# jydu/comap

Measured on AMD Instinct MI355X. Metric: site-pair coevolution statistics/s (incl. null sims), higher is better.
Workload: dtype f64; 1 GPU; target: north-star target: 10000x64 protein JTT92+G4(a=0.5), correlation, 1000 null replicates x 10000; observed_pairs=49995000, null_pairs_total=10000000, null_pairs_this_gpu=10000000, parallelism=single GPU, pair_output=compact, cu_count=256, mapping_waves=2048

## Files before the change

### comap_amd/csrc/cmx_api_ctx.cpp

```cpp
#include "cmx_ctx.h"

thread_local std::string g_create_error;

constexpr int kGuardByte = 0xC5;
std::atomic<int> g_guard{-1};
std::mutex g_guard_mu;
std::vector<std::string> g_guard_failures;
std::map<std::string, size_t> g_guard_shrink;

std::atomic<int> g_lds_slot{1};
std::atomic<int> g_pat_hash_bits{64};
std::atomic<int> g_map_queue{1};
std::atomic<int> g_map_small_blocks{1};
std::atomic<int> g_map_grid{0};

bool guard_on() {
  int g = g_guard.load();
  if (g < 0) {
    const char* e = getenv("CMX_SCRATCH_GUARD");
    g = (e && e[0] == '1') ? 1 : 0;
    g_guard.store(g);
  }
  return g == 1;
}

void guard_record(const std::string& what) {
  std::lock_guard<std::mutex> lk(g_guard_mu);
  g_guard_failures.push_back(what);
  std::fprintf(stderr, "CMX_SCRATCH_GUARD: %s\n", what.c_str());
}

hipError_t guard_arm(void* base, size_t logical) {
  return hipMemset(static_cast<char*>(base) + logical, kGuardByte, kGuardBytes);
}

bool guard_intact(const void* base, size_t logical, size_t* first_bad) {
// ... 173 lines not shown
      CMX_TRY(upload(ctx, h.MAT, &mat));
      d.MAT = const_cast<double*>(mat);
      d.MC = h.MC;
      auto up_stream = [&](const std::vector<int>& stream, const int** dev, int* nmv) -> cmx_status {
        std::vector<int> ms(stream);
        const int unit = mat_unit(h.dS);
        for (size_t i = 0; i < ms.size(); i += 2) ms[i] *= unit;
        const size_t n2 = ms.size();
        for (size_t i = 0; i < 4; ++i) ms.push_back(ms[i % n2]);
        *nmv = (int)(stream.size() / 2);
        return upload(ctx, ms, dev);
      };
      CMX_TRY(up_stream(h.msched, &d.msched, &d.nmv));
      d.msched_r = nullptr;
      d.nmv_r = 0;
      if (!h.msched_r.empty()) CMX_TRY(up_stream(h.msched_r, &d.msched_r, &d.nmv_r));
      d.plan = nullptr;
      if (!h.wait_imm.empty()) CMX_TRY(upload(ctx, planned_stream(h), &d.plan));
      UP(nrec);
    }
    UP(simg); UP(simord);
    d.nsimg = (int)(h.simg.size() / 16);
    UP(eigV); UP(eigVi); UP(eigLam); UP(model_of); UP(blen);
    UP(CP); UP(CPG); UP(pi); UP(rates); UP(probs); UP(cum_pi); UP(cum_probs);
#undef UP
    if (h.plain) return CMX_OK;
    HIP_TRY(ctx, launch_extend_leaf_rows(d, nullptr, nullptr));
    HIP_TRY(ctx, hipDeviceSynchronize());
    ctx->leaf_rows_custom = false;
    for (int i = 0; i < 256; ++i) dm[i] = i < h.S ? (1u << i) : ((h.S >= 32) ? 0xffffffffu : ((1u << h.S) - 1u));
    HIP_TRY(ctx, hipMemcpy(ctx->d_default_masks, dm.data(), sizeof(uint32_t) * 256, hipMemcpyHostToDevice));
    ctx->grid_blocks = ctx->cu_count * map_waves_per_simd(h.dS);
    ctx->waves = ctx->grid_blocks * kWavesPerBlock;
    ctx->obs_blocks = std::max(1, ctx->grid_blocks / 4);
    if (const int cap = g_map_grid.load()) {
      ctx->grid_blocks = std::min(ctx->grid_blocks, cap);
      ctx->waves = ctx->grid_blocks * kWavesPerBlock;
      ctx->obs_blocks = std::min(ctx->obs_blocks, cap);
    }
    auto alloc_ws = [&](Workspace* ws, size_t w, size_t* bytes) -> cmx_status {
      const size_t ks = (size_t)map_sites_per_wave(h.dS);
      const size_t bD = w * h.NIW * h.dS * ks * sizeof(double);
      const size_t bC = w * 2 * h.B * h.K * ks * sizeof(double);
      const size_t bP = w * h.dC * h.B * h.K * ks * sizeof(double);
      const bool g = guard_on();
      auto one = [&](const char* nm, void** p, size_t bytes) -> cmx_status {
// ... 101 lines not shown
}

cmx_status cmx_debug_wait_plan(const cmx_model* model, const cmx_tree* tree, int32_t* distance, int32_t* immediate, size_t cap, size_t* n) {
  HostModel hm;
  int code = CMX_OK;
  hm.lds_slot = g_lds_slot.load() != 0;
  const std::string msg = build_host_model(model, tree, &hm, &code);
  if (!msg.empty()) {
    g_create_error = msg;
    return (cmx_status)code;
  }
  if (hm.wait_imm.size() > cap) {
    g_create_error = "cmx_debug_wait_plan: buffers too small";
    return CMX_ERR_INVALID;
  }
  std::memcpy(distance, hm.wait_dist.data(), hm.wait_dist.size() * sizeof(int32_t));
  std::memcpy(immediate, hm.wait_imm.data(), hm.wait_imm.size() * sizeof(int32_t));
  *n = hm.wait_imm.size();
  return CMX_OK;
}

int cmx_debug_wait_skew(int entry) { return wait_plan_skew(entry); }

cmx_status cmx_synchronize(cmx_ctx* ctx) {
  if (!ctx) return CMX_ERR_INVALID;
  HIP_TRY(ctx, hipSetDevice(ctx->device));
  HIP_TRY(ctx, hipDeviceSynchronize());
  return guard_verify_all(ctx);
}

cmx_status cmx_scratch_check(cmx_ctx* ctx) {
  if (!ctx) return CMX_ERR_INVALID;
  if (!guard_on()) return fail(ctx, CMX_ERR_UNSUPPORTED, "the scratch guard is off (CMX_SCRATCH_GUARD=1 or cmx_debug_scratch_guard(1) before the context is created)");
  HIP_TRY(ctx, hipSetDevice(ctx->device));
  HIP_TRY(ctx, hipDeviceSynchronize());
  return guard_verify_all(ctx);
}

int cmx_debug_scratch_guard(int on) {
  const int was = guard_on() ? 1 : 0;
  if (on >= 0) g_guard.store(on ? 1 : 0);
  return was;
}

int cmx_debug_lds_slot(int on) {
  const int was = g_lds_slot.load();
  if (on >= 0) g_lds_slot.store(on ? 1 : 0);
  return was;
}

int cmx_debug_map_queue(int on) {
  const int was = g_map_queue.load();
  if (on >= 0) g_map_queue.store(on ? 1 : 0);
  return was;
}

int cmx_debug_map_small_blocks(int on) {
  const int was = g_map_small_blocks.load();
  if (on >= 0) g_map_small_blocks.store(on ? 1 : 0);
  return was;
}

int cmx_debug_map_grid(int workgroups) {
  const int was = g_map_grid.load();
  if (workgroups >= 0) g_map_grid.store(workgroups);
  return was;
}

size_t cmx_debug_scratch_guard_failures(char* buf, size_t cap, int clear) {
  std::lock_guard<std::mutex> lk(g_guard_mu);
  const size_t n = g_guard_failures.size();
  if (buf && cap) {
    std::string all;
    for (const std::string& f : g_guard_failures) { all += f; all += '\n'; }
    std::snprintf(buf, cap, "%s", all.c_str());
  }
// ... 78 lines not shown
```

### comap_amd/csrc/cmx_api_null.cpp

```cpp
#include "cmx_ctx.h"

constexpr size_t kNullAlnPassBytes = (size_t)4 << 30;
static size_t null_pass_bytes(size_t dflt) {
  static const size_t env = [] {
    const char* e = getenv("CMX_NULL_PASS_BYTES");
    return e ? (size_t)strtoull(e, nullptr, 10) : (size_t)0;
  }();
  return env ? env : dflt;
}

cmx_status cmx_null_simulate_dev(cmx_ctx* ctx, uint64_t seed, size_t rep_begin, size_t rep_end, size_t rep_ram, uint8_t* d_aln,
                                 void* stream) {
  CMX_TRY(need_model(ctx));
  if (rep_end <= rep_begin || rep_ram == 0 || !d_aln) return fail(ctx, CMX_ERR_INVALID, "cmx_null_simulate: bad arguments");
  CMX_TRY(rng_range(ctx, (uint64_t)rep_end * 2 * rep_ram, "cmx_null_simulate"));
  HIP_TRY(ctx, hipSetDevice(ctx->device));
  const size_t nsites = (rep_end - rep_begin) * 2 * rep_ram;
  const size_t chunk = std::min<size_t>(nsites, std::max<size_t>((size_t)1 << 21, (((size_t)4 << 30) / (size_t)ctx->hm.nn) & ~(size_t)1023));
  uint8_t* d_states;
  CMX_TRY(scratch(ctx, "null_states", (size_t)ctx->hm.nn * chunk, &d_states));
  HIP_TRY(ctx, launch_simulate_blocked(ctx->dm, seed, (uint64_t)rep_begin * 2 * rep_ram, nsites, rep_ram, d_aln, d_states, chunk,
                                       (hipStream_t)stream));
  return CMX_OK;
}

static cmx_status null_unfused_dev(cmx_ctx* ctx1, cmx_ctx* ctx2, int kind, const double* params, uint64_t seed,
                                   size_t rep_begin, size_t rep_end, size_t rep_ram, const uint8_t* d_supplied, double* d_stat,
                                   int32_t* d_rcmin, double* d_prmin, double* d_nmin, void* stream) {
  CMX_TRY(need_model(ctx1));
  if (!ctx2 || !ctx2->has_model) return fail(ctx1, CMX_ERR_INVALID, "cmx_null_inter: second context has no model");
  CMX_TRY(check_kind(ctx1, kind));
  if (rep_end <= rep_begin || rep_ram == 0 || !d_stat) return fail(ctx1, CMX_ERR_INVALID, "cmx_null_inter: bad arguments");
  CMX_TRY(rng_range(ctx1, (uint64_t)rep_end * 2 * rep_ram, "cmx_null_inter"));
  CMX_TRY(rng_range(ctx2, (uint64_t)rep_end * 2 * rep_ram, "cmx_null_inter"));
  if (ctx1->device != ctx2->device) return fail(ctx1, CMX_ERR_INVALID, "cmx_null_inter: contexts live on different devices");
  if (ctx1->hm.B != ctx2->hm.B || ctx1->hm.K != ctx2->hm.K)
    return fail(ctx1, CMX_ERR_INVALID, "cmx_null_inter: the two data sets must have the same branches and substitution types "
                                       "(Statistic::getValueForPair throws DimensionException otherwise)");
  HIP_TRY(ctx1, hipSetDevice(ctx1->device));
  hipStream_t st = (hipStream_t)stream;
  const size_t nrep = rep_end - rep_begin, n = nrep * rep_ram;
  const size_t BK = (size_t)ctx1->hm.B * ctx1->hm.K;
  double *cnt[2], *pr[2], *nm[2];
  int32_t* rc[2];
  cmx_ctx* cx[2] = {ctx1, ctx2};
// ... 261 lines not shown
```

### comap_amd/csrc/cmx_ctx.h

```cpp
#pragma once
#include <hip/hip_runtime.h>

#include <algorithm>
#include <atomic>
#include <cmath>
#include <cstdio>
#include <cstring>
#include <map>
#include <mutex>
#include <string>
#include <vector>

#include "../../include/comap_mi355x.h"
#include "cmx_device.h"
#include "cmx_host_model.h"

using namespace cmx;

#pragma GCC visibility push(hidden)

struct DevBuf {
  void* p = nullptr;
  size_t bytes = 0;
  size_t logical = 0;
// ... 5 lines not shown
  std::vector<long long> host;
  size_t M = 0;
  int sh = -1;
  size_t allocs = 0;
};

struct cmx_ctx {
  int device = 0;
  bool has_model = false;
  HostModel hm;
  DevModel dm{};
  Workspace ws{};
  Workspace ws_obs{};
  int obs_blocks = 0;
  int cu_count = 0, waves = 0, grid_blocks = 0;
  size_t ws_bytes = 0;
  unsigned long long* map_queue = nullptr;
  unsigned map_queue_turn = 0;
  std::vector<void*> model_allocs;
  std::map<std::string, DevBuf> scratch;
  struct GuardedFixed { std::string name; void* p; size_t bytes; };
  std::vector<GuardedFixed> guarded_fixed;
  uint32_t* d_default_masks = nullptr;
  unsigned stat_mean_turn = 0;
  std::vector<double> param_host[8];
  bool leaf_rows_custom = false;
  bool map_average = true;
  bool map_joint = true;
  bool scaling = false;
  std::vector<double> stat_w;
  double* d_stat_w = nullptr;
  std::vector<long long> perm_dF_host;
  std::vector<uint8_t> perm_tab_host;
  PermTable perm_F, permw_F;
  struct GramKept { bool valid = false; int kind = 0; const double* counts = nullptr; size_t n = 0, ldc = 0, row_begin = 0, row_end = 0; const double* stat = nullptr; } gram_kept;
  const double *va_P = nullptr, *va_N1 = nullptr, *va_NC = nullptr;
  const double *va_PN = nullptr, *va_pi = nullptr;
  const int *va_first = nullptr, *va_next = nullptr;
  WideOps va_wide{};
  const int* asr_inner = nullptr;
  int asr_n_inner = 0;
  int null_patterns = -1;
  int null_depth = 0;
  unsigned long long null_mapped_host = 0;
  bool null_mapped_dev = false;
  mutable std::string err;
// ... 2 lines not shown
#define CMX_TRY(expr)                                                                                        \
  do {                                                                                                       \
    cmx_status s_ = (expr);                                                                                  \
    if (s_ != CMX_OK) return s_;                                                                             \
  } while (0)

#define HIP_TRY(ctx, expr)                                                                                   \
  do {                                                                                                       \
    hipError_t e_ = (expr);                                                                                  \
    if (e_ != hipSuccess) {                                                                                  \
      (ctx)->err = std::string(#expr) + ": " + hipGetErrorString(e_);                                        \
      return CMX_ERR_DEVICE;                                                                                 \
    }                                                                                                        \
  } while (0)

extern thread_local std::string g_create_error;
extern std::atomic<int> g_guard;
extern std::mutex g_guard_mu;
extern std::vector<std::string> g_guard_failures;
extern std::map<std::string, size_t> g_guard_shrink;
extern std::atomic<int> g_pat_hash_bits;
extern std::atomic<int> g_map_queue;
extern std::atomic<int> g_map_small_blocks;
extern std::atomic<int> g_map_grid;

inline cmx_status fail(cmx_ctx* ctx, cmx_status s, const std::string& msg) {
  if (ctx) ctx->err = msg;
  return s;
}

inline cmx_status need_model(cmx_ctx* ctx) {
  if (!ctx) return CMX_ERR_INVALID;
  if (!ctx->has_model) return fail(ctx, CMX_ERR_INVALID, "this context was created without a model/tree");
  return CMX_OK;
}

template <class T>
cmx_status upload(cmx_ctx* ctx, const std::vector<T>& h, const T** d) {
  void* p = nullptr;
  const size_t bytes = sizeof(T) * (h.empty() ? 1 : h.size());
  HIP_TRY(ctx, hipMalloc(&p, bytes));
  ctx->model_allocs.push_back(p);
  if (!h.empty()) HIP_TRY(ctx, hipMemcpy(p, h.data(), sizeof(T) * h.size(), hipMemcpyHostToDevice));
  *d = static_cast<const T*>(p);
  return CMX_OK;
}
// ... 94 lines not shown
```

### comap_amd/csrc/cmx_device.h

```cpp
#pragma once
#include <hip/hip_runtime.h>

#include "../../include/comap_mi355x.h"
#include <stddef.h>
#include <stdint.h>

#include "cmx_layout.h"

namespace cmx {

constexpr int kWave = 64;
constexpr int kWavesPerBlock = 4;
constexpr int map_ng(int) { return 4; }
constexpr int map_sites_per_wave(int S) { return 16 * map_ng(S); }
constexpr int map_waves_per_simd(int S) { return S == 4 ? 3 : 2; }
constexpr bool map_lds_slot(int S, int fuse, int ng) { return S == 20 && fuse == 1 && ng == 4; }

struct DevModel {
  int S, C, K, nn, B, T, NI, NIW, NV, root;
  int S0, C0, fuse;
  const int* taxon_of;
  const int* parent;
  double* MAT;
  int MC;
// ... 92 lines not shown
inline int pair_Bp(int B) { return (B + 3) / 4 * 4; }
struct SiteCols { const int32_t* rc = nullptr; const double *pr = nullptr, *nm = nullptr; };
struct PairOut {
  double* stat = nullptr;
  int32_t* rcmin = nullptr;
  double *prmin = nullptr, *nmin = nullptr;
  PairOut at(size_t o) const { return {stat + o, rcmin ? rcmin + o : nullptr, prmin ? prmin + o : nullptr, nmin ? nmin + o : nullptr}; }
};
struct GramBatch { size_t nblk, zsite, zout, zx; };
struct RowScan { unsigned long long* rowcount = nullptr; void* tmp = nullptr; size_t tmp_bytes = 0; };

hipError_t launch_map(const MapArgs& a, int mode, int grid_blocks, hipStream_t stream);
hipError_t launch_map_queue_init(unsigned long long* queue, unsigned long long first, hipStream_t stream);
hipError_t launch_map_finalize(const MapArgs& a, hipStream_t stream);
hipError_t launch_extend_leaf_rows(const DevModel& m, const uint32_t* d_masks, hipStream_t stream);
hipError_t launch_pair_diag(const Stat& st, const double* c1, size_t ld1, const SiteCols& s1, const double* c2, size_t ld2,
                            const SiteCols& s2, size_t n, const PairOut& out, hipStream_t stream);
hipError_t launch_group_stats(const Stat& st, const double* d_counts, size_t ld, const int64_t* d_offsets, const int32_t* d_sites,
                              size_t ngroups, double* d_out, hipStream_t stream);
hipError_t launch_simulate(const DevModel& m, uint64_t seed, uint64_t g0, size_t n, uint8_t* d_aln, size_t ld,
                           int32_t* d_classes, uint8_t* d_states, hipStream_t stream, size_t rep_ram = 0, uint64_t gstep = 0);
hipError_t launch_simulate_continuous(const DevModel& m, uint64_t seed, uint64_t g0, size_t n, double alpha, double p_inv,
                                      uint8_t* d_aln, size_t ld, double* d_rates, uint8_t* d_states, hipStream_t stream);
hipError_t launch_simulate_blocked(const DevModel& m, uint64_t seed, uint64_t g0, size_t nsites, size_t blk, uint8_t* d_aln,
                                   uint8_t* d_states, size_t chunk, hipStream_t stream);
hipError_t launch_pair_prep(const Stat& st, const double* d_counts, size_t n, size_t ldc, const double* d_mvec, size_t blk,
                            const PairOperand& o, hipStream_t stream);
hipError_t launch_pair_gram(const Stat& st, const PairOperand& a, const PairOperand& b, PairMode mode, double* d_out, size_t ldo,
                            const GramBatch& z, size_t irow0, hipStream_t stream);
hipError_t launch_mi_classify(const Stat& st, const double* d_counts, size_t n, size_t ldc, const PairOperand& o, hipStream_t stream);
hipError_t launch_mi_pairs_block(int B, const PairOperand& a, const PairOperand& b, PairMode mode, double* d_out, size_t ldo,
                                 size_t irow0, hipStream_t stream);
hipError_t launch_mi_pairs_diag(int B, const PairOperand& a, const PairOperand& b, size_t n, double* d_out, hipStream_t stream);
hipError_t launch_mi_group(int B, const PairOperand& g, const int64_t* d_offsets, const int32_t* d_sites, size_t ngroups,
                           double* d_out, hipStream_t stream);
enum class PlainMode : int { NoAvg = 0 , Marginal = 1, NoAvgMarginal = 2 , Joint = 3 };
struct PlainArgs {
  int S, C, K, nn, B, root;
  PlainMode mode;
  int Sreal;
  const double* PN;
  const double* rates;
  double *logL, *post_rate;
  int32_t* rate_class;
  const int *first_child, *next_sib, *taxon_of, *parent;
  const double* P;
  const double* N1;
  const double* NC;
// ... 166 lines not shown
```

### comap_amd/csrc/cmx_host_model.cpp

```cpp
#include "cmx_host_parts.h"

#include <algorithm>
#include <cmath>
#include <cstring>

namespace cmx {
namespace {

using Mat = std::vector<double>;

Mat matmul(int n, const Mat& A, const Mat& B) {
  Mat C((size_t)n * n, 0.0);
  for (int i = 0; i < n; ++i)
    for (int k = 0; k < n; ++k) {
      const double a = A[(size_t)i * n + k];
      for (int j = 0; j < n; ++j) C[(size_t)i * n + j] += a * B[(size_t)k * n + j];
    }
  return C;
}

void jacobi(int n, Mat A, Mat* U, std::vector<double>* lam) {
  U->assign((size_t)n * n, 0.0);
  for (int i = 0; i < n; ++i) (*U)[(size_t)i * n + i] = 1.0;
  for (int sweep = 0; sweep < 200; ++sweep) {
// ... 308 lines not shown

void build_sim_tables(HostModel* hm) {
  const int S = hm->S, C = hm->C, B = hm->B, nn = hm->nn;
  const size_t S2 = (size_t)S * S;
  hm->CP.assign((size_t)C * nn * S2 + 4, 0.0);
  for (int c = 0; c < C; ++c)
    for (int b = 0; b < B; ++b) {
      const double* P = &hm->P[((size_t)c * B + b) * S2];
      double* cp = &hm->CP[((size_t)c * nn + b) * S2];
      for (int x = 0; x < S; ++x) {
        double cum = 0.0;
        for (int y = 0; y < S; ++y) { cum += P[(size_t)x * S + y]; cp[(size_t)x * S + y] = cum; }
      }
    }
  hm->CPG.assign((size_t)C * nn * S * 32, 0);
  for (size_t r = 0; r < (size_t)C * nn * S; ++r) {
    const double* cum = &hm->CP[r * S];
    for (int k = 0; k < 32; ++k) {
      int st = 0;
      while (st < S - 1 && cum[st] <= k / 32.0) ++st;
      hm->CPG[r * 32 + k] = (uint8_t)st;
    }
  }
  hm->cum_pi.resize(S);
  hm->cum_probs.resize(C);
  double cum = 0.0;
  for (int x = 0; x < S; ++x) { cum += hm->pi[x]; hm->cum_pi[x] = cum; }
  cum = 0.0;
  for (int c = 0; c < C; ++c) { cum += hm->probs[c]; hm->cum_probs[c] = cum; }
}

}

std::string build_host_model(const cmx_model* model, const cmx_tree* tree, HostModel* hm, int* code) {
  *code = CMX_ERR_INVALID;
  std::vector<Eig> eig;
  std::string bad = check_arguments(model, tree, hm, code);
  if (bad.empty()) bad = build_tree(tree, hm);
  if (!bad.empty()) return bad;
  build_walk_program(hm);
  build_sim_groups(hm);
  bad = check_model(model, hm);
  if (bad.empty()) bad = build_generators(model, hm, &eig);
  if (!bad.empty()) return bad;
  build_branch_matrices(model, eig, hm);
  build_device_matrices(hm);
// ... 10 lines not shown
```

### comap_amd/csrc/cmx_host_model.h

```cpp
#pragma once
#include <cstdint>
#include <string>
#include <vector>

#include "../../include/comap_mi355x.h"
#include "cmx_layout.h"

namespace cmx {

struct HostModel {
  int S = 0, C = 0, K = 0, nn = 0, B = 0, T = 0, NI = 0, root = 0;
  int dS = 0, dC = 0, fuse = 1;
  bool plain = false;
  std::vector<int> parent, first_child, next_sib, taxon_of, slot, int_post;
  std::vector<double> blen, pi, rates, probs, cum_pi, cum_probs;
  std::vector<double> P;
  std::vector<double> PN;
  std::vector<double> N1;
  std::vector<double> NC;
  std::vector<double> MAT;
  int MC = 0;
  std::vector<double> eigV, eigVi, eigLam;
  std::vector<int> model_of;
  std::vector<double> CP;
  std::vector<uint8_t> CPG;
  std::vector<int> simg;
  std::vector<int> simord;
  int NV = 0;
  int NIW = 0;
  std::vector<int> nrec;
  std::vector<int> msched;
  std::vector<int> ldsched;
  std::vector<int> wait_dist, wait_imm;
  std::vector<int> cherry_of;
  int ncherry = 0, cherry_base = 0;
  std::vector<int> msched_r;
  ClassBlock block() const { return {NI, K, T, ncherry}; }
  size_t n_loads = 0, n_stores = 0, n_products = 0, n_leaf_ops = 0, n_products_r = 0, n_leaf_ops_r = 0;
  bool lds_slot = true;
  size_t n_lds_loads = 0, n_lds_stores = 0, n_lds_copies = 0;
};

void build_records(HostModel* hm);
void plan_lds_slot(HostModel* hm);
void record_walk(HostModel* hm);
std::string verify_walk(const HostModel& hm);
std::vector<PlanEntry> planned_stream(const HostModel& hm);
int wait_plan_skew(int entry);
// ... 5 lines not shown
```

### comap_amd/csrc/cmx_layout.h

```cpp
#pragma once

namespace cmx {

constexpr int kPlainStates = 64;

constexpr int max_ambig(int S) { return S == 4 ? 12 : 4; }
constexpr int leaf_row_stride(int S) { return S + 1; }
constexpr int mat_unit(int S) { return (S + max_ambig(S)) * leaf_row_stride(S); }
constexpr int leaf_col(int X, int dS) { return (X % 4) * (dS / 4) + X / 4; }

constexpr int mfma_a_tile_offset(int lane, bool tr) {
  return (tr ? 4 * (lane >> 4) + (lane & 3) : 4 * (lane & 3) + (lane >> 4)) * 8;
}
constexpr int mfma16_a_offset(int lane, int i, bool tr, int S) {
  return ((tr ? i * (S / 4) + ((lane & 15) >> 2) : ((lane & 15) >> 2) * (S / 4) + i) * 16) * 8 + mfma_a_tile_offset(lane, tr);
}

constexpr int wide_op_offset(int row, int col, int S = kPlainStates) {
  return ((row >> 4) * (S / 4) + (col >> 2)) * 64 + (col & 3) * 16 + (row & 15);
}
constexpr bool wide_op_offset_is_bijection() {
  bool seen[kPlainStates * kPlainStates] = {};
  for (int r = 0; r < kPlainStates; ++r)
    for (int c = 0; c < kPlainStates; ++c) {
      const int o = wide_op_offset(r, c);
      if (o < 0 || o >= kPlainStates * kPlainStates || seen[o]) return false;
      seen[o] = true;
// ... 76 lines not shown
```

### comap_amd/csrc/cmx_simulate.hip

```cpp
#include <algorithm>

#include "cmx_device.h"
#include "cmx_lanes.h"

namespace cmx {

__device__ __forceinline__ void philox_words(uint64_t seed, uint64_t g, uint32_t draw, uint32_t& w0, uint32_t& w1) {
  uint32_t c0 = (uint32_t)g, c1 = ((uint32_t)(g >> 32) & 0x7fffu) | (draw << 15);
  uint32_t k = (uint32_t)seed ^ ((uint32_t)(seed >> 32) * 0x9E3779B9u) ^ 0x434d5832u;
#pragma unroll
  for (int r = 0; r < 10; ++r) {
    const uint64_t p = (uint64_t)0xD256D193u * (uint64_t)c0;
    c0 = __builtin_amdgcn_bitop3_b32((uint32_t)(p >> 32), k, c1, 0x96);
    c1 = (uint32_t)p;
    k += 0x9E3779B9u;
  }
  w0 = c0;
  w1 = c1;
}
__device__ __forceinline__ double philox_uniform(uint64_t seed, uint64_t g, uint32_t draw) {
  uint32_t c0, c1;
  philox_words(seed, g, draw, c0, c1);
  const uint64_t bits = (((uint64_t)c0 << 32) | c1) >> 11;
  return (double)bits * (1.0 / 9007199254740992.0);
// ... 217 lines not shown
        *reinterpret_cast<unsigned short*>(sn + (unsigned)j[k]) = (unsigned short)(idx[k] | (idx[k + 1] << 8));
        if (tx >= 0) {
          if (((blk | (size_t)(uintptr_t)aln) & 1) == 0) {
            *reinterpret_cast<unsigned short*>(out[k] + (size_t)tx * blk) = (unsigned short)(idx[k] | (idx[k + 1] << 8));
          } else {
            out[k][(size_t)tx * blk] = (uint8_t)idx[k];
            out[k + 1][(size_t)tx * blk] = (uint8_t)idx[k + 1];
          }
        }
      }
    if (more) {
      __syncthreads();
#pragma unroll
      for (int i = 0; i < NCH; ++i) {
        const int q = tid + NT * i;
        if (q < nch && q * 16 < tabb + guib) reinterpret_cast<cmx_i4*>(sim_smem + (size_t)(buf ^ 1) * bufb)[q] = nxt[i];
      }
      __syncthreads();
      buf ^= 1;
    }
  }
}

constexpr size_t kSimLdsMinSites = 450000;
hipError_t launch_simulate_blocked(const DevModel& m, uint64_t seed, uint64_t g0, size_t nsites, size_t blk, uint8_t* d_aln,
                                   uint8_t* d_states, size_t chunk, hipStream_t stream) {
  const size_t bufb = ((size_t)m.C0 * m.S0 * (m.S0 * 8 + 32) + 15) & ~(size_t)15;
  const bool lds = m.S0 > 4 && bufb <= (size_t)kSimLdsChunks * 256 * 16;
  for (size_t s0 = 0; s0 < nsites; s0 += chunk) {
    const size_t n = std::min(chunk, nsites - s0);
    if (lds && n >= kSimLdsMinSites && (g0 & 1) == 0 && (s0 & 1) == 0 && (n & 1) == 0) {
      if (bufb <= (size_t)2 * 512 * 16)
        hipLaunchKernelGGL((simulate_lds_kernel<2, 2, 512, 8>), dim3((unsigned)((n + 1023) / 1024)), dim3(512), 2 * bufb, stream, m, seed, g0, s0,
                           n, blk, d_aln, d_states);
      else
        hipLaunchKernelGGL((simulate_lds_kernel<4, kSimLdsChunks, 256, 4>), dim3((unsigned)((n + 1023) / 1024)), dim3(256), 2 * bufb, stream, m,
                           seed, g0, s0, n, blk, d_aln, d_states);
    }
    else
      hipLaunchKernelGGL(simulate_blocked_kernel, dim3((unsigned)((n + 255) / 256)), dim3(256), 0, stream, m, seed, g0, s0, n, blk,
                         d_aln, d_states);
  }
  return hipGetLastError();
}


__host__ __device__ inline void cmx_gamma_pq(double a, double x, double* p, double* q) {
  if (x <= 0.0) { *p = 0.0; *q = 1.0; return; }
  const double pre = exp(-x + a * log(x) - lgamma(a));
  if (x < a + 1.0) {
    double term = 1.0 / a, sum = term;
    for (int n = 1; n < 1000; ++n) {
      term *= x / (a + n);
      sum += term;
      if (fabs(term) < fabs(sum) * 1e-17) break;
// ... 88 lines not shown
```

### comap_amd/engine.py

```python
import ctypes
import os

import numpy as np

_HERE = os.path.dirname(os.path.abspath(__file__))
LIB_PATH = os.environ.get("COMAP_MI355X_LIB", os.path.join(_HERE, "libcomap_mi355x.so"))

STAT_CORRELATION, STAT_COMPENSATION, STAT_COSUBSTITUTION, STAT_COSINUS, STAT_COVARIANCE, STAT_DISCRETE_MI, \
    STAT_CORRECTED_CORRELATION, STAT_EUCLIDIAN_DISTANCE, STAT_DISCRETE_MI_BOUNDS, STAT_SCALAR_PRODUCT = range(10)
STAT_BY_NAME = {
    "Correlation": STAT_CORRELATION, "Compensation": STAT_COMPENSATION, "Cosubstitution": STAT_COSUBSTITUTION,
    "Cosinus": STAT_COSINUS, "Covariance": STAT_COVARIANCE, "MI": STAT_DISCRETE_MI,
    "CorrectedCorrelation": STAT_CORRECTED_CORRELATION, "EuclidianDistance": STAT_EUCLIDIAN_DISTANCE,
    "MI(bounds)": STAT_DISCRETE_MI_BOUNDS,
}


def label_mi_bounds(nstates):
    n = nstates * (nstates - 1)
    return -0.5 + np.arange(n + 2, dtype=np.float64)


def _stat_params(kind, threshold, mean_vectors):
    if int(kind) == STAT_CORRECTED_CORRELATION:
# ... 1 lines not shown
            raise CmxError(-1, "CorrectedCorrelation needs mean_vectors")
        mv = _f64(mean_vectors)
        if mv.ndim == 1:
            mv = np.stack([mv, mv])
        return np.ascontiguousarray(mv)
    if int(kind) == STAT_DISCRETE_MI_BOUNDS:
        b = _f64(threshold).ravel()
        return np.ascontiguousarray(np.concatenate([[float(len(b))], b]))
    return _f64([threshold])
COUNT_EXPECTED, COUNT_NAIVE = 0, 1

EXPORTS = [
    "cmx_version", "cmx_ctx_create", "cmx_ctx_destroy", "cmx_last_error", "cmx_get_info",
    "cmx_get_transition_matrices", "cmx_synchronize", "cmx_debug_walk", "cmx_map_sites", "cmx_set_mapping_options", "cmx_set_likelihood_scaling", "cmx_get_likelihood_scaling", "cmx_set_statistic_weights", "cmx_get_statistic_weights", "cmx_map_sites_dev", "cmx_ancestral_states", "cmx_ancestral_states_dev", "cmx_simulate", "cmx_simulate_dev", "cmx_simulate_continuous",
    "cmx_simulate_continuous_dev", "cmx_null_intra_continuous", "cmx_null_intra_continuous_dev", "cmx_mi_pairs_dev",
    "cmx_pair_stats", "cmx_pair_stats_dev", "cmx_null_intra", "cmx_null_simulate_dev", "cmx_null_intra_dev", "cmx_null_inter",
    "cmx_null_inter_dev", "cmx_intra_pvalues", "cmx_intra_rows", "cmx_intra_rows_dev", "cmx_intra_rows_range_dev",
    "cmx_intra_pvalues_dev", "cmx_inter_rows", "cmx_inter_rows_dev", "cmx_mica_bootstrap_indices", "cmx_mica_parametric_null", "cmx_mi_columns", "cmx_mi_columns_dev", "cmx_mi_pairs", "cmx_debug_mica_wide_plain", "cmx_debug_map_wide_plain", "cmx_debug_map_scaled_plain",
    "cmx_mica_permutation_test", "cmx_mica_permutation_test_dev", "cmx_mica_permutation_test_masks", "cmx_mica_permutation_test_masks_dev", "cmx_mica_permutation_test_states", "cmx_mica_permutation_test_states_dev", "cmx_mica_average_mi", "cmx_mica_average_mi_dev", "cmx_mica_zscore_null", "cmx_mica_zscore_null_dev",
    "cmx_group_stats", "cmx_group_stats_dev", "cmx_candidate_groups", "cmx_debug_candidate_cursor",
    "cmx_hclust", "cmx_hclust_dev", "cmx_cluster_sites", "cmx_cluster_sites_dev", "cmx_cluster_null",
    "cmx_intra_compact_range_dev", "cmx_intra_gram_prefetch_dev", "cmx_expand_compact_rows", "cmx_vector_matrix",
    "cmx_scratch_check", "cmx_debug_lds_slot", "cmx_debug_map_queue", "cmx_debug_map_grid", "cmx_debug_scratch_guard", "cmx_debug_scratch_guard_failures", "cmx_debug_scratch_shrink",
    "cmx_set_null_patterns", "cmx_null_pattern_count", "cmx_debug_null_hash_bits", "cmx_debug_wait_plan", "cmx_debug_wait_skew", "cmx_debug_map_small_blocks",
]
DIST_CORRELATION, DIST_COMPENSATION, DIST_EUCLIDIAN = range(3)
LINK_COMPLETE, LINK_SINGLE, LINK_AVERAGE = range(3)
DIST_BY_NAME = {"cor": DIST_CORRELATION, "Correlation": DIST_CORRELATION, "comp": DIST_COMPENSATION,
                "Compensation": DIST_COMPENSATION, "euclidian": DIST_EUCLIDIAN, "Euclidian": DIST_EUCLIDIAN}
LINK_BY_NAME = {"complete": LINK_COMPLETE, "single": LINK_SINGLE, "average": LINK_AVERAGE}
CLUSTER_MAX_SITES = 5000
MICA_MI, MICA_MIP, MICA_MIC = range(3)


def scratch_guard(on=None):
    lib = load_library()
    return bool(lib.cmx_debug_scratch_guard(ctypes.c_int(-1 if on is None else int(bool(on)))))


def lds_slot(on=None):
    lib = load_library()
    return bool(lib.cmx_debug_lds_slot(ctypes.c_int(-1 if on is None else int(bool(on)))))


def map_queue(on=None):
    lib = load_library()
    return bool(lib.cmx_debug_map_queue(ctypes.c_int(-1 if on is None else int(bool(on)))))


def map_small_blocks(on=None):
    lib = load_library()
    return bool(lib.cmx_debug_map_small_blocks(ctypes.c_int(-1 if on is None else int(bool(on)))))


def map_grid(workgroups=None):
    lib = load_library()
    return int(lib.cmx_debug_map_grid(ctypes.c_int(-1 if workgroups is None else int(workgroups))))


def mica_wide_plain(on=None):
    lib = load_library()
    return bool(lib.cmx_debug_mica_wide_plain(ctypes.c_int(-1 if on is None else int(bool(on)))))


def map_wide_plain(on=None):
    lib = load_library()
    return bool(lib.cmx_debug_map_wide_plain(ctypes.c_int(-1 if on is None else int(bool(on)))))


def map_scaled_plain(on=None):
# ... 160 lines not shown
    return dict(nrec=nrec[: n1.value].reshape(-1, 16).copy(), ldsched=ld[: n2.value].copy(),
                msched=ms[: n3.value].reshape(-1, 2).copy(), slot=slot, loads=int(stats[0]), stores=int(stats[1]),
                products=int(stats[2]), leaf_ops=int(stats[3]), products_tables=int(stats[4]), leaf_ops_tables=int(stats[5]),
                cherry_tables=int(stats[6]), lds_loads=int(stats[7]) & 0xfffff, lds_stores=(int(stats[7]) >> 20) & 0xfffff,
                lds_copies=(int(stats[7]) >> 40) & 0xfffff)


def debug_wait_plan(parent, blen, leaf_of_taxon, Q, pi, rates, probs, Bk=None):
    lib = load_library()
    keep = [np.ascontiguousarray(parent, dtype=np.int32), _f64(blen), np.ascontiguousarray(leaf_of_taxon, dtype=np.int32),
            _f64(Q), _f64(pi), _f64(rates), _f64(probs), None if Bk is None else _f64(Bk)]
    p, bl, lot, Qa, pia, ra, pr, Bka = keep
    S, C = len(pia), len(ra)
    K = 1 if Bka is None else Bka.reshape(-1, S, S).shape[0]
    model = _Model(S, C, K, _vp(Qa), _vp(pia), _vp(ra), _vp(pr), _vp(Bka), 0, 1, _vp(None))
    tree = _Tree(len(p), _vp(p), _vp(bl), len(lot), _vp(lot))
    cap = 64 * len(p) * max(K, 1) + 64
    dist, imm = np.zeros(cap, dtype=np.int32), np.zeros(cap, dtype=np.int32)
    n = ctypes.c_size_t(0)
    st = lib.cmx_debug_wait_plan(ctypes.byref(model), ctypes.byref(tree), _vp(dist), _vp(imm), _sz(cap), ctypes.byref(n))
    if st != 0:
        raise CmxError(st, lib.cmx_last_error(None).decode())
    return dict(distance=dist[: n.value].copy(), immediate=imm[: n.value].copy())


def wait_skew(entry=None):
    lib = load_library()
    return int(lib.cmx_debug_wait_skew(ctypes.c_int(-1 if entry is None else int(entry))))


def debug_candidate_cursor(norm_windows, analysable, min_sim, norms, max_trials):
    lib = load_library()
    off = np.zeros(len(norm_windows) + 1, dtype=np.int64)
    off[1:] = np.cumsum([len(g) for g in norm_windows])
    lo = _f64([w[0] for g in norm_windows for w in g])
    hi = _f64([w[1] for g in norm_windows for w in g])
    ok = np.ascontiguousarray(analysable, dtype=np.uint8)
    nm = _f64(norms)
    nb, rr = nm.shape
    G = len(norm_windows)
    n2 = np.zeros(G, dtype=np.uint32)
    cap = nb * rr
    pg_group, pg_batch = np.zeros(cap, dtype=np.int32), np.zeros(cap, dtype=np.int32)
    pg_off, pg_sites = np.zeros(cap + 1, dtype=np.int64), np.zeros(cap, dtype=np.int32)
    trials, used, npg = ctypes.c_uint32(0), ctypes.c_uint64(0), ctypes.c_size_t(0)
    st = lib.cmx_debug_candidate_cursor(_sz(G), _vp(off), _vp(lo), _vp(hi), _vp(ok), ctypes.c_uint32(min_sim), _vp(nm), _sz(rr),
# ... 523 lines not shown
```

### include/comap_mi355x.h

```cpp
#ifndef COMAP_MI355X_H
#define COMAP_MI355X_H

#include <stddef.h>
#include <stdint.h>

#ifdef __cplusplus
extern "C" {
#endif

typedef struct cmx_ctx cmx_ctx;

typedef enum {
  CMX_OK = 0,
  CMX_ERR_INVALID = -1,
  CMX_ERR_UNSUPPORTED = -2,
  CMX_ERR_DEVICE = -3,
  CMX_ERR_NOMEM = -4,
  CMX_ERR_INTERNAL = -5
} cmx_status;

typedef enum {
  CMX_STAT_CORRELATION = 0,
  CMX_STAT_COMPENSATION = 1,
  CMX_STAT_COSUBSTITUTION = 2,
// ... 50 lines not shown

const char* cmx_version(void);
cmx_status cmx_ctx_create(const cmx_model* model, const cmx_tree* tree, int device, cmx_ctx** out);
void cmx_ctx_destroy(cmx_ctx* ctx);
const char* cmx_last_error(const cmx_ctx* ctx);
cmx_status cmx_get_info(const cmx_ctx* ctx, cmx_info* info);
cmx_status cmx_get_transition_matrices(const cmx_ctx* ctx, double* P);
cmx_status cmx_synchronize(cmx_ctx* ctx);
cmx_status cmx_scratch_check(cmx_ctx* ctx);
int cmx_debug_scratch_guard(int on);
size_t cmx_debug_scratch_guard_failures(char* buf, size_t cap, int clear);
void cmx_debug_scratch_shrink(const char* name, size_t bytes);
cmx_status cmx_debug_walk(const cmx_model* model, const cmx_tree* tree, int32_t* nrec, size_t nrec_cap, size_t* nrec_n,
                          int32_t* ldsched, size_t ld_cap, size_t* ld_n, int32_t* msched, size_t m_cap, size_t* m_n,
                          int32_t* slot_of_node ,
                          uint64_t* stats );
cmx_status cmx_debug_wait_plan(const cmx_model* model, const cmx_tree* tree, int32_t* distance, int32_t* immediate, size_t cap,
                               size_t* n);
int cmx_debug_wait_skew(int entry);
int cmx_debug_lds_slot(int on);
int cmx_debug_map_queue(int on);
int cmx_debug_map_grid(int workgroups);
int cmx_debug_map_small_blocks(int on);

cmx_status cmx_map_sites(cmx_ctx* ctx, const uint8_t* aln, size_t nsites, size_t ld, const uint32_t* masks,
                         size_t nmasks, double* counts , double* logL, double* post_rate,
                         int32_t* rate_class, double* norm);
cmx_status cmx_map_sites_dev(cmx_ctx* ctx, const uint8_t* d_aln, size_t nsites, size_t ld, const uint32_t* d_masks,
                             double* d_counts , size_t ldc, double* d_logL, double* d_post_rate,
                             int32_t* d_rate_class, double* d_norm, void* stream);
int cmx_debug_map_wide_plain(int on);
int cmx_debug_map_scaled_plain(int on);
cmx_status cmx_set_mapping_options(cmx_ctx* ctx, int average, int joint);
cmx_status cmx_set_likelihood_scaling(cmx_ctx* ctx, int on);
cmx_status cmx_get_likelihood_scaling(const cmx_ctx* ctx, int32_t* on);

cmx_status cmx_ancestral_states(cmx_ctx* ctx, const uint8_t* aln, size_t nsites, size_t ld, const uint32_t* masks, size_t nmasks,
                                uint8_t* states , double* post );
cmx_status cmx_ancestral_states_dev(cmx_ctx* ctx, const uint8_t* d_aln, size_t nsites, size_t ld, const uint32_t* d_masks,
                                    uint8_t* d_states, size_t lds, double* d_post, size_t ldp, void* stream);

cmx_status cmx_set_statistic_weights(cmx_ctx* ctx, const double* w, size_t nbranches);
cmx_status cmx_get_statistic_weights(const cmx_ctx* ctx, double* w_out, int32_t* has_weights);

cmx_status cmx_simulate(cmx_ctx* ctx, uint64_t seed, uint64_t g0, size_t n, uint8_t* aln_out, int32_t* classes_out);
cmx_status cmx_simulate_dev(cmx_ctx* ctx, uint64_t seed, uint64_t g0, size_t n, uint8_t* d_aln, size_t ld, int32_t* d_classes,
// ... 190 lines not shown
```

Measured before the change: 221.5 million site-pair statistics/s.

## Add chained null-simulation kernel with precomputed uint32 thresholds and per-node LDS tables

Precomputes, per tree node, a compact table of 32-bit integer cumulative thresholds plus guide bytes on the host and uploads it once. A new simulation kernel double-buffers each node's table in LDS, compares raw Philox words against integer thresholds in multi-step searches instead of doubles, and keeps the child state in registers when the next node's parent is the current node, skipping a global reload. Large chunks use a four-batch-per-thread variant. The trade-off is extra host table construction and memory, plus slightly different sampling boundaries from the integer threshold rounding.

```diff
diff --git a/comap_amd/csrc/cmx_api_ctx.cpp b/comap_amd/csrc/cmx_api_ctx.cpp
--- a/comap_amd/csrc/cmx_api_ctx.cpp
+++ b/comap_amd/csrc/cmx_api_ctx.cpp
@@ -12,6 +12,9 @@
 std::atomic<int> g_pat_hash_bits{64};
 std::atomic<int> g_map_queue{1};
 std::atomic<int> g_map_small_blocks{1};
+std::atomic<int> g_sim_chain{1};
+std::atomic<long long> g_sim_lds_min_sites{-1};
+std::atomic<long long> g_sim_four_batch_sites{-1};
 std::atomic<int> g_map_grid{0};
 
 bool guard_on() {
@@ -231,6 +234,8 @@
     UP(simg); UP(simord);
     d.nsimg = (int)(h.simg.size() / 16);
     UP(eigV); UP(eigVi); UP(eigLam); UP(model_of); UP(blen);
+    ctx->d_simtab = nullptr;
+    if (!h.simtab.empty()) CMX_TRY(upload(ctx, h.simtab, &ctx->d_simtab));
     UP(CP); UP(CPG); UP(pi); UP(rates); UP(probs); UP(cum_pi); UP(cum_probs);
 #undef UP
     if (h.plain) return CMX_OK;
@@ -378,6 +383,29 @@
 
 int cmx_debug_wait_skew(int entry) { return wait_plan_skew(entry); }
 
+cmx_status cmx_debug_sim_tables(const cmx_model* model, const cmx_tree* tree, double* cum, size_t cum_cap, uint8_t* guide,
+                                size_t guide_cap, uint8_t* blocks, size_t blocks_cap, size_t* blocks_bytes, int32_t* row) {
+  HostModel hm;
+  int code = CMX_OK;
+  const std::string msg = build_host_model(model, tree, &hm, &code);
+  if (!msg.empty()) {
+    g_create_error = msg;
+    return (cmx_status)code;
+  }
+  const size_t ncum = (size_t)hm.C * hm.nn * hm.S * hm.S, nguide = (size_t)hm.C * hm.nn * hm.S * 32;
+  if (blocks_bytes) *blocks_bytes = hm.simtab.size();
+  if (row) *row = sim_thr_row(hm.S);
+  if (!cum && !guide && !blocks) return CMX_OK;
+  if (!cum || !guide || !blocks || cum_cap < ncum || guide_cap < nguide || blocks_cap < hm.simtab.size()) {
+    g_create_error = "cmx_debug_sim_tables: a buffer is missing or too small";
+    return CMX_ERR_INVALID;
+  }
+  std::memcpy(cum, hm.CP.data(), ncum * sizeof(double));
+  std::memcpy(guide, hm.CPG.data(), nguide);
+  if (!hm.simtab.empty()) std::memcpy(blocks, hm.simtab.data(), hm.simtab.size());
+  return CMX_OK;
+}
+
 cmx_status cmx_synchronize(cmx_ctx* ctx) {
   if (!ctx) return CMX_ERR_INVALID;
   HIP_TRY(ctx, hipSetDevice(ctx->device));
@@ -408,6 +436,14 @@
 int cmx_debug_map_queue(int on) {
   const int was = g_map_queue.load();
   if (on >= 0) g_map_queue.store(on ? 1 : 0);
+  return was;
+}
+
+int cmx_debug_sim_chain(int on, long long min_sites, long long four_batch_sites) {
+  const int was = g_sim_chain.load();
+  if (on >= 0) g_sim_chain.store(on ? 1 : 0);
+  if (min_sites >= -1) g_sim_lds_min_sites.store(min_sites);
+  if (four_batch_sites >= -1) g_sim_four_batch_sites.store(four_batch_sites);
   return was;
 }
 
diff --git a/comap_amd/csrc/cmx_api_null.cpp b/comap_amd/csrc/cmx_api_null.cpp
--- a/comap_amd/csrc/cmx_api_null.cpp
+++ b/comap_amd/csrc/cmx_api_null.cpp
@@ -19,8 +19,9 @@
   const size_t chunk = std::min<size_t>(nsites, std::max<size_t>((size_t)1 << 21, (((size_t)4 << 30) / (size_t)ctx->hm.nn) & ~(size_t)1023));
   uint8_t* d_states;
   CMX_TRY(scratch(ctx, "null_states", (size_t)ctx->hm.nn * chunk, &d_states));
+  const SimChoice choice{ctx->d_simtab, g_sim_chain.load() != 0, g_sim_lds_min_sites.load(), g_sim_four_batch_sites.load()};
   HIP_TRY(ctx, launch_simulate_blocked(ctx->dm, seed, (uint64_t)rep_begin * 2 * rep_ram, nsites, rep_ram, d_aln, d_states, chunk,
-                                       (hipStream_t)stream));
+                                       (hipStream_t)stream, choice));
   return CMX_OK;
 }
 
diff --git a/comap_amd/csrc/cmx_ctx.h b/comap_amd/csrc/cmx_ctx.h
--- a/comap_amd/csrc/cmx_ctx.h
+++ b/comap_amd/csrc/cmx_ctx.h
@@ -51,6 +51,7 @@
   struct GuardedFixed { std::string name; void* p; size_t bytes; };
   std::vector<GuardedFixed> guarded_fixed;
   uint32_t* d_default_masks = nullptr;
+  const uint8_t* d_simtab = nullptr;
   unsigned stat_mean_turn = 0;
   std::vector<double> param_host[8];
   bool leaf_rows_custom = false;
@@ -99,6 +100,9 @@
 extern std::atomic<int> g_pat_hash_bits;
 extern std::atomic<int> g_map_queue;
 extern std::atomic<int> g_map_small_blocks;
+extern std::atomic<int> g_sim_chain;
+extern std::atomic<long long> g_sim_lds_min_sites;
+extern std::atomic<long long> g_sim_four_batch_sites;
 extern std::atomic<int> g_map_grid;
 
 inline cmx_status fail(cmx_ctx* ctx, cmx_status s, const std::string& msg) {
diff --git a/comap_amd/csrc/cmx_device.h b/comap_amd/csrc/cmx_device.h
--- a/comap_amd/csrc/cmx_device.h
+++ b/comap_amd/csrc/cmx_device.h
@@ -138,8 +138,14 @@
                            int32_t* d_classes, uint8_t* d_states, hipStream_t stream, size_t rep_ram = 0, uint64_t gstep = 0);
 hipError_t launch_simulate_continuous(const DevModel& m, uint64_t seed, uint64_t g0, size_t n, double alpha, double p_inv,
                                       uint8_t* d_aln, size_t ld, double* d_rates, uint8_t* d_states, hipStream_t stream);
+struct SimChoice {
+  const uint8_t* simtab;
+  bool chain;
+  long long lds_min_sites;
+  long long four_batch_sites;
+};
 hipError_t launch_simulate_blocked(const DevModel& m, uint64_t seed, uint64_t g0, size_t nsites, size_t blk, uint8_t* d_aln,
-                                   uint8_t* d_states, size_t chunk, hipStream_t stream);
+                                   uint8_t* d_states, size_t chunk, hipStream_t stream, const SimChoice& choice);
 hipError_t launch_pair_prep(const Stat& st, const double* d_counts, size_t n, size_t ldc, const double* d_mvec, size_t blk,
                             const PairOperand& o, hipStream_t stream);
 hipError_t launch_pair_gram(const Stat& st, const PairOperand& a, const PairOperand& b, PairMode mode, double* d_out, size_t ldo,
diff --git a/comap_amd/csrc/cmx_host_model.cpp b/comap_amd/csrc/cmx_host_model.cpp
--- a/comap_amd/csrc/cmx_host_model.cpp
+++ b/comap_amd/csrc/cmx_host_model.cpp
@@ -354,6 +354,26 @@
       hm->CPG[r * 32 + k] = (uint8_t)st;
     }
   }
+  hm->simtab.clear();
+  if (S > 4 && sim_node_bytes(S, C) <= kSimNodeBytesMax) {
+    const int rs = sim_thr_row(S);
+    const size_t nodeb = sim_node_bytes(S, C), tabb = (size_t)C * S * rs * 4;
+    hm->simtab.assign((size_t)nn * nodeb, 0);
+    for (int b = 0; b < B; ++b)
+      for (int c = 0; c < C; ++c)
+        for (int x = 0; x < S; ++x) {
+          const size_t r = ((size_t)c * nn + b) * S + x;
+          uint32_t thr[kPlainStates + kSimThrPad + 3];
+          for (int y = 0; y < rs; ++y) {
+            const double t = y < S - 1 ? std::ceil(std::ldexp(hm->CP[r * S + y], 32)) - 1.0 : 4294967295.0;
+            thr[y] = t <= 0.0 ? 0u : t >= 4294967295.0 ? 0xffffffffu : (uint32_t)t;
+            if (y > 0) thr[y] = std::max(thr[y], thr[y - 1]);
+          }
+          uint8_t* node = &hm->simtab[(size_t)b * nodeb];
+          std::memcpy(node + ((size_t)c * S + x) * rs * 4, thr, (size_t)rs * 4);
+          std::memcpy(node + tabb + ((size_t)c * S + x) * 32, &hm->CPG[r * 32], 32);
+        }
+  }
   hm->cum_pi.resize(S);
   hm->cum_probs.resize(C);
   double cum = 0.0;
diff --git a/comap_amd/csrc/cmx_host_model.h b/comap_amd/csrc/cmx_host_model.h
--- a/comap_amd/csrc/cmx_host_model.h
+++ b/comap_amd/csrc/cmx_host_model.h
@@ -24,6 +24,7 @@
   std::vector<int> model_of;
   std::vector<double> CP;
   std::vector<uint8_t> CPG;
+  std::vector<uint8_t> simtab;
   std::vector<int> simg;
   std::vector<int> simord;
   int NV = 0;
diff --git a/comap_amd/csrc/cmx_layout.h b/comap_amd/csrc/cmx_layout.h
--- a/comap_amd/csrc/cmx_layout.h
+++ b/comap_amd/csrc/cmx_layout.h
@@ -3,6 +3,11 @@
 namespace cmx {
 
 constexpr int kPlainStates = 64;
+
+constexpr int kSimThrPad = 4;
+constexpr int sim_thr_row(int S) { return (S + kSimThrPad + 3) & ~3; }
+constexpr unsigned long sim_node_bytes(int S, int C) { return (unsigned long)C * S * (sim_thr_row(S) * 4 + 32); }
+constexpr unsigned long kSimNodeBytesMax = 3ul * 512 * 16;
 
 constexpr int max_ambig(int S) { return S == 4 ? 12 : 4; }
 constexpr int leaf_row_stride(int S) { return S + 1; }
diff --git a/comap_amd/csrc/cmx_simulate.hip b/comap_amd/csrc/cmx_simulate.hip
--- a/comap_amd/csrc/cmx_simulate.hip
+++ b/comap_amd/csrc/cmx_simulate.hip
@@ -263,15 +263,153 @@
   }
 }
 
+template <int NB , int NCH , int NT, int WAVES, int STEP>
+__global__ __launch_bounds__(NT) __attribute__((amdgpu_waves_per_eu(WAVES, WAVES))) void simulate_chain_kernel(const DevModel m, const uint8_t* __restrict__ tabs, uint64_t seed, uint64_t g0, size_t s0, size_t n,
+                                                           size_t blk, uint8_t* __restrict__ aln, uint8_t* __restrict__ states) {
+  static_assert(STEP <= kSimThrPad, "a search reads STEP thresholds past its index");
+  extern __shared__ __attribute__((aligned(16))) uint8_t sim_smem[];
+  const int S0 = m.S0, C0 = m.C0, tid = threadIdx.x;
+  const int rs = sim_thr_row(S0), tabb = C0 * S0 * rs * 4, nodeb = (int)sim_node_bytes(S0, C0), nch = nodeb / 16;
+  const size_t jb0 = (size_t)blockIdx.x * NB * (2 * NT) + (size_t)(2 * tid);
+  const uint64_t gp0 = (g0 + s0 + jb0) >> 1;
+  uint8_t* out[NB];
+  unsigned crow[NB], xc[NB];
+  unsigned on = 0, wrap = 0;
+#pragma unroll
+  for (int b = 0; b < NB; ++b) {
+    const size_t jj = jb0 + (size_t)b * (2 * NT);
+    const bool in = jj < n;
+    const size_t s = s0 + (in ? jj : 0);
+    const uint64_t g = g0 + s;
+    const size_t col = s % blk;
+    out[b] = aln + (s / blk) * (size_t)m.T * blk + col;
+    on |= (in ? 1u : 0u) << b;
+    wrap |= (col == blk - 1 ? 1u : 0u) << b;
+    const int c0 = draw_index(philox_uniform(seed, g, 0), m.cum_probs, C0), c1 = draw_index(philox_uniform(seed, g + 1, 0), m.cum_probs, C0);
+    crow[b] = (unsigned)(c0 * S0) | ((unsigned)(c1 * S0) << 16);
+    const int r0 = draw_index(philox_uniform(seed, g, 1), m.cum_pi, S0), r1 = draw_index(philox_uniform(seed, g + 1, 1), m.cum_pi, S0);
+    xc[b] = (unsigned)r0 | ((unsigned)r1 << 8);
+    if (in) *reinterpret_cast<unsigned short*>(states + (size_t)m.root * n + jj) = (unsigned short)xc[b];
+  }
+  const cmx_cint ord = (cmx_cint)m.simord;
+  int buf = 0;
+  for (int q = tid; q < nch; q += NT)
+    reinterpret_cast<cmx_i4*>(sim_smem)[q] = reinterpret_cast<const cmx_i4*>(tabs + (size_t)ord[0] * nodeb)[q];
+  __syncthreads();
+  for (int it = 0; it < m.nn - 1; ++it) {
+    const int node = ord[it];
+    const bool more = it + 1 < m.nn - 1;
+    cmx_i4 nxt[NCH];
+    unsigned xn[NB];
+    bool chain = false;
+    if (more) {
+      const int nnode = ord[it + 1], npar = ((cmx_cint)m.parent)[nnode];
+      const cmx_i4* src = reinterpret_cast<const cmx_i4*>(tabs + (size_t)nnode * nodeb);
+#pragma unroll
+      for (int i = 0; i < NCH; ++i)
+        if (tid + NT * i < nch) nxt[i] = src[tid + NT * i];
+      chain = npar == node;
+      if (!chain) {
+        const uint8_t* sp = states + (size_t)npar * n + (unsigned)jb0;
+#pragma unroll
+        for (int b = 0; b < NB; ++b) xn[b] = (on >> b & 1) ? *reinterpret_cast<const unsigned short*>(sp + b * (2 * NT)) : 0u;
+      }
+    }
+    const uint32_t* T_ = reinterpret_cast<const uint32_t*>(sim_smem + (size_t)buf * nodeb);
+    const uint8_t* G_ = sim_smem + (size_t)buf * nodeb + tabb;
+    const int tx = ((cmx_cint)m.taxon_of)[node];
+    uint8_t* sn = states + (size_t)node * n + (unsigned)jb0;
+#pragma unroll
+    for (int b = 0; b < NB; ++b) {
+      uint32_t w[2];
+      philox_words(seed, gp0 + (uint64_t)(b * NT), 2u + (uint32_t)node, w[0], w[1]);
+      int idx[2];
+      const uint32_t* thr[2];
+#pragma unroll
+      for (int k = 0; k < 2; ++k) {
+        const int row = (int)((crow[b] >> (16 * k)) & 0xffffu) + (int)((xc[b] >> (8 * k)) & 0xffu);
+        idx[k] = G_[row * 32 + (int)(w[k] >> 27)];
+        thr[k] = T_ + __mul24(row, rs);
+      }
+      bool any;
+      do {
+        uint32_t tv[2][STEP];
+#pragma unroll
+        for (int k = 0; k < 2; ++k)
+#pragma unroll
+          for (int d = 0; d < STEP; ++d) tv[k][d] = thr[k][idx[k] + d];
+        any = false;
+#pragma unroll
+        for (int k = 0; k < 2; ++k) {
+          int adv = 0;
+#pragma unroll
+          for (int d = 0; d < STEP; ++d) adv += w[k] > tv[k][d] ? 1 : 0;
+          idx[k] += adv;
+          any |= adv == STEP;
+        }
+      } while (any);
+      const unsigned pair = (unsigned)idx[0] | ((unsigned)idx[1] << 8);
+      if (chain) xn[b] = pair;
+      if (on >> b & 1) {
+        if (tx < 0) {
+          *reinterpret_cast<unsigned short*>(sn + b * (2 * NT)) = (unsigned short)pair;
+        } else if (((blk | (size_t)(uintptr_t)aln) & 1) == 0) {
+          *reinterpret_cast<unsigned short*>(out[b] + (size_t)tx * blk) = (unsigned short)pair;
+        } else {
+          uint8_t* o = out[b] + (size_t)tx * blk;
+          o[0] = (uint8_t)idx[0];
+          o[(wrap >> b & 1) ? 1 + (size_t)(m.T - 1) * blk : (size_t)1] = (uint8_t)idx[1];
+        }
+      }
+    }
+    if (more) {
+#pragma unroll
+      for (int b = 0; b < NB; ++b) xc[b] = xn[b];
+#pragma unroll
+      for (int i = 0; i < NCH; ++i)
+        if (tid + NT * i < nch) reinterpret_cast<cmx_i4*>(sim_smem + (size_t)(buf ^ 1) * nodeb)[tid + NT * i] = nxt[i];
+      __syncthreads();
+      buf ^= 1;
+    }
+  }
+}
+
+constexpr size_t kSimChainMinSites = 75000;
 constexpr size_t kSimLdsMinSites = 450000;
+constexpr size_t kSimChainFourBatches = (size_t)4 * 1024 * 1024;
 hipError_t launch_simulate_blocked(const DevModel& m, uint64_t seed, uint64_t g0, size_t nsites, size_t blk, uint8_t* d_aln,
-                                   uint8_t* d_states, size_t chunk, hipStream_t stream) {
+                                   uint8_t* d_states, size_t chunk, hipStream_t stream, const SimChoice& choice) {
   const size_t bufb = ((size_t)m.C0 * m.S0 * (m.S0 * 8 + 32) + 15) & ~(size_t)15;
   const bool lds = m.S0 > 4 && bufb <= (size_t)kSimLdsChunks * 256 * 16;
+  const uint8_t* d_simtab = choice.simtab;
+  const size_t nodeb = sim_node_bytes(m.S0, m.C0);
+  const bool chain = lds && d_simtab && nodeb <= kSimNodeBytesMax && choice.chain;
+  const size_t min_sites = choice.lds_min_sites >= 0 ? (size_t)choice.lds_min_sites : chain ? kSimChainMinSites : kSimLdsMinSites;
+  const size_t four_sites = choice.four_batch_sites >= 0 ? (size_t)choice.four_batch_sites : kSimChainFourBatches;
   for (size_t s0 = 0; s0 < nsites; s0 += chunk) {
     const size_t n = std::min(chunk, nsites - s0);
-    if (lds && n >= kSimLdsMinSites && (g0 & 1) == 0 && (s0 & 1) == 0 && (n & 1) == 0) {
-      if (bufb <= (size_t)2 * 512 * 16)
+    if (lds && n >= min_sites && (g0 & 1) == 0 && (s0 & 1) == 0 && (n & 1) == 0) {
+      if (chain) {
+        const bool two = nodeb <= (size_t)2 * 512 * 16;
+        if (n >= four_sites) {
+          const dim3 grid((unsigned)((n + 4095) / 4096));
+          if (two)
+            hipLaunchKernelGGL((simulate_chain_kernel<4, 2, 512, 8, 2>), grid, dim3(512), 2 * nodeb, stream, m, d_simtab, seed, g0, s0, n, blk,
+                               d_aln, d_states);
+          else
+            hipLaunchKernelGGL((simulate_chain_kernel<4, 3, 512, 8, 2>), grid, dim3(512), 2 * nodeb, stream, m, d_simtab, seed, g0, s0, n, blk,
+                               d_aln, d_states);
+        } else {
+          const dim3 grid((unsigned)((n + 1023) / 1024));
+          if (two)
+            hipLaunchKernelGGL((simulate_chain_kernel<1, 2, 512, 8, 4>), grid, dim3(512), 2 * nodeb, stream, m, d_simtab, seed, g0, s0, n, blk,
+                               d_aln, d_states);
+          else
+            hipLaunchKernelGGL((simulate_chain_kernel<1, 3, 512, 8, 4>), grid, dim3(512), 2 * nodeb, stream, m, d_simtab, seed, g0, s0, n, blk,
+                               d_aln, d_states);
+        }
+      }
+      else if (bufb <= (size_t)2 * 512 * 16)
         hipLaunchKernelGGL((simulate_lds_kernel<2, 2, 512, 8>), dim3((unsigned)((n + 1023) / 1024)), dim3(512), 2 * bufb, stream, m, seed, g0, s0,
                            n, blk, d_aln, d_states);
       else
diff --git a/comap_amd/engine.py b/comap_amd/engine.py
--- a/comap_amd/engine.py
+++ b/comap_amd/engine.py
@@ -47,7 +47,7 @@
     "cmx_hclust", "cmx_hclust_dev", "cmx_cluster_sites", "cmx_cluster_sites_dev", "cmx_cluster_null",
     "cmx_intra_compact_range_dev", "cmx_intra_gram_prefetch_dev", "cmx_expand_compact_rows", "cmx_vector_matrix",
     "cmx_scratch_check", "cmx_debug_lds_slot", "cmx_debug_map_queue", "cmx_debug_map_grid", "cmx_debug_scratch_guard", "cmx_debug_scratch_guard_failures", "cmx_debug_scratch_shrink",
-    "cmx_set_null_patterns", "cmx_null_pattern_count", "cmx_debug_null_hash_bits", "cmx_debug_wait_plan", "cmx_debug_wait_skew", "cmx_debug_map_small_blocks",
+    "cmx_set_null_patterns", "cmx_null_pattern_count", "cmx_debug_null_hash_bits", "cmx_debug_wait_plan", "cmx_debug_wait_skew", "cmx_debug_map_small_blocks", "cmx_debug_sim_chain", "cmx_debug_sim_tables",
 ]
 DIST_CORRELATION, DIST_COMPENSATION, DIST_EUCLIDIAN = range(3)
 LINK_COMPLETE, LINK_SINGLE, LINK_AVERAGE = range(3)
@@ -71,6 +71,13 @@
 def map_queue(on=None):
     lib = load_library()
     return bool(lib.cmx_debug_map_queue(ctypes.c_int(-1 if on is None else int(bool(on)))))
+
+
+def sim_chain(on=None, min_sites=None, four_batch_sites=None):
+    lib = load_library()
+    return bool(lib.cmx_debug_sim_chain(ctypes.c_int(-1 if on is None else int(bool(on))),
+                                        ctypes.c_longlong(-2 if min_sites is None else int(min_sites)),
+                                        ctypes.c_longlong(-2 if four_batch_sites is None else int(four_batch_sites))))
 
 
 def map_small_blocks(on=None):
@@ -277,6 +284,36 @@
     if st != 0:
         raise CmxError(st, lib.cmx_last_error(None).decode())
     return dict(distance=dist[: n.value].copy(), immediate=imm[: n.value].copy())
+
+
+def debug_sim_tables(parent, blen, leaf_of_taxon, Q, pi, rates, probs):
+    lib = load_library()
+    keep = [np.ascontiguousarray(parent, dtype=np.int32), _f64(blen), np.ascontiguousarray(leaf_of_taxon, dtype=np.int32),
+            _f64(Q), _f64(pi), _f64(rates), _f64(probs)]
+    p, bl, lot, Qa, pia, ra, pr = keep
+    S, C, nn = len(pia), len(ra), len(p)
+    model = _Model(S, C, 1, _vp(Qa), _vp(pia), _vp(ra), _vp(pr), _vp(None), 0, 1, _vp(None))
+    tree = _Tree(nn, _vp(p), _vp(bl), len(lot), _vp(lot))
+    nbytes, row = ctypes.c_size_t(0), ctypes.c_int32(0)
+
+    def call(cum, guide, blocks):
+        st = lib.cmx_debug_sim_tables(ctypes.byref(model), ctypes.byref(tree), _vp(cum), _sz(0 if cum is None else cum.size),
+                                      _vp(guide), _sz(0 if guide is None else guide.size), _vp(blocks),
+                                      _sz(0 if blocks is None else blocks.size), ctypes.byref(nbytes), ctypes.byref(row))
+        if st != 0:
+            raise CmxError(st, lib.cmx_last_error(None).decode())
+    call(None, None, None)
+    cum, guide = np.zeros((C, nn, S, S)), np.zeros((C, nn, S, 32), dtype=np.uint8)
+    blocks = np.zeros(max(nbytes.value, 1), dtype=np.uint8)
+    call(cum, guide, blocks)
+    R = row.value
+    out = dict(cum=cum, guide=guide, row=R, thresholds=None, block_guide=None)
+    if nbytes.value:
+        assert nbytes.value == nn * C * S * (4 * R + 32)
+        b = blocks.reshape(nn, C * S * (4 * R + 32))
+        out["thresholds"] = b[:, : C * S * 4 * R].copy().view(np.uint32).reshape(nn, C, S, R)
+        out["block_guide"] = b[:, C * S * 4 * R:].reshape(nn, C, S, 32).copy()
+    return out
 
 
 def wait_skew(entry=None):
diff --git a/include/comap_mi355x.h b/include/comap_mi355x.h
--- a/include/comap_mi355x.h
+++ b/include/comap_mi355x.h
@@ -96,6 +96,9 @@
 int cmx_debug_map_queue(int on);
 int cmx_debug_map_grid(int workgroups);
 int cmx_debug_map_small_blocks(int on);
+int cmx_debug_sim_chain(int on, long long min_sites, long long four_batch_sites);
+cmx_status cmx_debug_sim_tables(const cmx_model* model, const cmx_tree* tree, double* cum, size_t cum_cap, uint8_t* guide,
+                                size_t guide_cap, uint8_t* blocks, size_t blocks_cap, size_t* blocks_bytes, int32_t* row);
 
 cmx_status cmx_map_sites(cmx_ctx* ctx, const uint8_t* aln, size_t nsites, size_t ld, const uint32_t* masks,
                          size_t nmasks, double* counts , double* logL, double* post_rate,
```

Result: faster. 225.0 million site-pair statistics/s, median of 6 (+1.6%).
